# VITA-Group/SinNeRF

Measured on NVIDIA H100. Metric: rays/sec (64c+64f samples, 8x256 MLP), higher is better.
Workload: dtype fp32-parity: fp16 hi/lo split x3 on wgmma, fp32 accumulate

## Files before the change

### sinnerf_b200/csrc/field_tc.cu

```cuda
#include <stddef.h>
#include <stdlib.h>

#include <type_traits>
#include <utility>

#include "act16.cuh"
#include "common.cuh"
#include "wgmma.cuh"

namespace snb {
using namespace wg;

constexpr int kTile = 128;
constexpr int kNh = 128;
constexpr int kKc = 32;
constexpr uint32_t kStepBytes = kNh * 16 * 2;
constexpr int kWgs = 2;
constexpr int kThreads = (kWgs + 1) * 128;
constexpr int kProducerRegs = 24, kConsumerRegs = 240;
static_assert(128 * kProducerRegs + kWgs * 128 * kConsumerRegs <= 65536, "register file");
constexpr size_t kSmemOptIn = 232448;

enum { SRC_ENC = 0, SRC_HID = 1, SRC_DIR = 2 };

// ... 361 lines not shown
};

template <bool kBf16, bool kSplit, bool kEmbedded, int kTrain = 0>
__global__ void __launch_bounds__(kThreads, 1) field_tc_kernel(TcParams p) {
  static_assert(!(kTrain != 0 && kEmbedded), "the training forward is the fused (rays, z) entry only");
  using Smem = TcSmem<kSplit>;
  extern __shared__ unsigned char smem_raw[];
  Smem& s = *reinterpret_cast<Smem*>((reinterpret_cast<uintptr_t>(smem_raw) + 127) & ~uintptr_t(127));
  constexpr ConstLayout CL = make_const_layout();
  constexpr int kStages = Smem::kStages;
  constexpr int kParts = Smem::kParts;
  const ChunkTable& tab = c_chunks;
  const int tid = threadIdx.x, warp = tid >> 5, lane = tid & 31;
  const PackedHeader* hdr = reinterpret_cast<const PackedHeader*>(p.image);
  const int new_activation = hdr->new_activation;
  const float* g_cst = reinterpret_cast<const float*>(p.image + sizeof(PackedHeader));
  const unsigned char* g_chunks = p.image + sizeof(PackedHeader) + kConstBytes;
  const long long ntiles = (p.n_points + kTile - 1) / kTile;
  const int n_chunks = p.sigma_only ? tab.n_sigma_only : tab.n_total;

  if (tid == 0) {
    for (int i = 0; i < kStages; ++i) { mbar_init(&s.full[i], 1); mbar_init(&s.empty[i], kWgs * 4); }
    fence_mbar_init();
  }
  __syncthreads();

  if (warp >= kWgs * 4) {
    setmaxnreg_dec<kProducerRegs>();
    if (warp == kWgs * 4 && elect_one()) {
      const long long my_tiles = ntiles > (long long)blockIdx.x ? (ntiles - 1 - blockIdx.x) / gridDim.x + 1 : 0;
      const long long n_loads = my_tiles * n_chunks;
      uint32_t st = 0, ph = 0;
      int ci = 0;
      for (long long i = 0; i < n_loads; ++i) {
        mbar_wait(&s.empty[st], ph ^ 1);
        const Chunk c = tab.c[ci];
        const uint32_t bytes = kStepBytes * kParts * c.steps;
        mbar_arrive_expect_tx(&s.full[st], bytes);
        bulk_g2s(s.ring[st], g_chunks + (size_t)c.off * (kStepBytes * kParts), bytes, &s.full[st]);
        if (++ci == n_chunks) ci = 0;
        if (++st == kStages) { st = 0; ph ^= 1; }
      }
    }
    return;
  }
  setmaxnreg_inc<kConsumerRegs>();

  const int wgi = warp >> 2, wq = warp & 3, tq = lane & 3;
  const int r0 = wgi * 64 + wq * 16 + (lane >> 2);
  auto wg_sync = [&]() { named_bar_sync(1 + wgi, 128); };
  constexpr uint32_t kHidPart = kTile * kWidth * 2, kEncPart = kTile * kXyzPad * 2;
  constexpr uint32_t kOffRing = offsetof(Smem, ring), kOffHid = offsetof(Smem, hid), kOffEnc = offsetof(Smem, enc);
  const uint32_t sbase = smem_u32(&s);
  const uint32_t a_wg = sbase + wgi * 64 * 16;
  const uint32_t hid_thr = sbase + kOffHid + r0 * 16 + tq * 4;
  const int er = wgi * 64 + (tid & 63), epart = (tid >> 6) & 1;

  auto store_cell16 = [&](unsigned char* base, long long pt, int f8, int F, const float (&v)[8]) SNB_INLINE {
    if (pt >= p.ppad) return;
    const bool live = pt < p.n_points;
    uint4 c;
    c.x = live ? pack_half2_sat(v[0], v[1]) : 0u; c.y = live ? pack_half2_sat(v[2], v[3]) : 0u;
    c.z = live ? pack_half2_sat(v[4], v[5]) : 0u; c.w = live ? pack_half2_sat(v[6], v[7]) : 0u;
    *reinterpret_cast<uint4*>(base + a16_cell(pt, f8, F)) = c;
  };

  struct RowIn { float4 q0, q1; float z; };
  RowIn in{};
  auto load_row = [&](long long tile) SNB_INLINE {
    const long long pt = tile * kTile + er;
    if (!kEmbedded && tile < ntiles && pt < p.n_points) {
      const long long ray = pt / p.n_samples;
      in.q0 = *reinterpret_cast<const float4*>(p.rays + ray * 8);
      in.q1 = *reinterpret_cast<const float4*>(p.rays + ray * 8 + 4);
      in.z = p.z[pt];
    }
  };
  auto encode = [&](auto ltag, auto ptag, long long tile) SNB_INLINE {
    constexpr int L = decltype(ltag)::value, P = decltype(ptag)::value;
    constexpr bool kXyz = L == SNB_XYZ_FREQS;
    constexpr int kCh = 3 * (2 * L + 1), kPad = (kCh + 7) / 8 * 8, kK8 = kPad / 16;
    constexpr int c_lo = 8 * kK8 * P, c_hi = 8 * kK8 * (P + 1);
    const long long pt = tile * kTile + er;
    const bool live = pt < p.n_points;
    float v[kPad];
#pragma unroll
    for (int j = 0; j < kPad; ++j) v[j] = 0.f;
    if (kEmbedded) {
      const float* xr = p.x + pt * p.x_stride;
      const int nin = p.sigma_only ? kXyzCh : kXyzCh + kDirCh;
#pragma unroll
      for (int j = c_lo; j < (c_hi < kCh ? c_hi : kCh); ++j) {
        const int col = kXyz ? j : kXyzCh + j;
        v[j] = (live && col < nin) ? xr[col] : 0.f;
      }
    } else {
      float x[3] = {0.f, 0.f, 0.f};
      if (live) {
        if (kXyz) {
          x[0] = __fadd_rn(in.q0.x, __fmul_rn(in.q0.w, in.z));
          x[1] = __fadd_rn(in.q0.y, __fmul_rn(in.q1.x, in.z));
          x[2] = __fadd_rn(in.q0.z, __fmul_rn(in.q1.y, in.z));
        } else {
          x[0] = in.q0.w; x[1] = in.q1.x; x[2] = in.q1.y;
        }
      }
      v[0] = x[0]; v[1] = x[1]; v[2] = x[2];
#pragma unroll
      for (int f = 0; f < L; ++f)
#pragma unroll
        for (int c = 0; c < 3; ++c) {
          const int cs = 3 + 6 * f + c, cc = cs + 3;
          if ((cs >= c_lo && cs < c_hi) || (cc >= c_lo && cc < c_hi)) {
            float sn, cs_;
            if (kSplit) sincosf(x[c] * (float)(1 << f), &sn, &cs_);
            else sincos_fast(x[c] * (float)(1 << f), &sn, &cs_);
            v[cs] = sn;
            v[cc] = cs_;
          }
        }
    }
    static_for<kK8>([&](auto ktag) SNB_INLINE {
      constexpr int k8 = kK8 * P + decltype(ktag)::value;
      const float v8[8] = {v[8 * k8], v[8 * k8 + 1], v[8 * k8 + 2], v[8 * k8 + 3], v[8 * k8 + 4], v[8 * k8 + 5], v[8 * k8 + 6], v[8 * k8 + 7]};
      if (!kEmbedded) {
        if (kTrain == 1 && live) {
          float4* dst = reinterpret_cast<float4*>((kXyz ? p.save_enc + pt * kXyzPad : p.save_dir + pt * kDirPad) + k8 * 8);
          dst[0] = make_float4(v8[0], v8[1], v8[2], v8[3]); dst[1] = make_float4(v8[4], v8[5], v8[6], v8[7]);
        }
        if (kTrain == 2) store_cell16(kXyz ? p.a_enc : p.a_dir, pt, k8, kXyz ? kXyzPad : kDirPad, v8);
      }
      uint32_t h[4], l[4];
#pragma unroll
      for (int j = 0; j < 4; ++j) split_pair<kBf16, kSplit>(v8[2 * j], v8[2 * j + 1], h[j], l[j]);
      const uint32_t a = sbase + kOffEnc + k8 * (kTile * 16) + er * 16;
      st_shared_v4(a, h[0], h[1], h[2], h[3]);
      if (kSplit) st_shared_v4(a + kEncPart, l[0], l[1], l[2], l[3]);
    });
  };
  auto encode_rows = [&](auto ltag, long long tile) SNB_INLINE {
    if (epart == 0) encode(ltag, std::integral_constant<int, 0>{}, tile);
    else encode(ltag, std::integral_constant<int, 1>{}, tile);
  };

  auto mma = [&](float (&d)[64], uint64_t a, uint64_t b, bool first) SNB_INLINE {
    if (first) {
      if (kBf16) wgmma_m64n128_bf16_first(d, a, b);
      else wgmma_m64n128_f16_first(d, a, b);
    } else {
      if (kBf16) wgmma_m64n128_bf16(d, a, b, 1u);
      else wgmma_m64n128_f16(d, a, b, 1u);
    }
  };
  auto issue_step = [&](float (&d)[64], uint32_t ah, uint32_t al, uint32_t bh, uint32_t bl, bool first) SNB_INLINE {
    const uint64_t da_h = make_smem_desc(ah, kTile * 16, 128), db_h = make_smem_desc(bh, kNh * 16, 128);
    mma(d, da_h, db_h, first);
    if (kSplit) {
      mma(d, make_smem_desc(al, kTile * 16, 128), db_h, false);
      mma(d, da_h, make_smem_desc(bl, kNh * 16, 128), false);
    }
  };

  constexpr bool kDrained = kTrain != 0;
  float acc[2][64];
  float sig[2] = {0.f, 0.f};

  uint32_t st = 0, ph = 0;
  auto prev_stage = [&]() { return st == 0 ? (uint32_t)kStages - 1 : st - 1; };
  auto issue = [&](auto ctag) SNB_INLINE {
    constexpr int ci = decltype(ctag)::value;
    constexpr Chunk c = h_chunks.c[ci];
    float (&d)[64] = acc[c.half];
    mbar_wait(&s.full[st], ph);
    wgmma_fence();
    const uint32_t bh = sbase + kOffRing + st * Smem::kStageBytes, bl = bh + kStepBytes * c.steps;
    uint32_t abase;
    asm volatile("mov.b32 %0, %1;" : "=r"(abase) : "r"(a_wg));
    const uint32_t ah = abase + (c.src == SRC_HID ? kOffHid : kOffEnc) + c.a16 * 2 * (kTile * 16);
    constexpr uint32_t part = c.src == SRC_HID ? kHidPart : kEncPart;
    static_for<c.steps>([&](auto ktag) SNB_INLINE {
      constexpr int ks = decltype(ktag)::value;
      issue_step(d, ah + ks * 2 * (kTile * 16), ah + ks * 2 * (kTile * 16) + part, bh + ks * kStepBytes,
                 bl + ks * kStepBytes, ks == 0 && c.first);
    });
    wgmma_commit();
    if (kDrained ? !(c.first && c.half == 0) : ci != 0) {
      wgmma_wait<1>();
      if (lane == 0) mbar_arrive(&s.empty[prev_stage()]);
      __syncwarp();
    }
    if (++st == kStages) { st = 0; ph ^= 1; }
  };
  auto issue_range = [&](auto c0tag, auto ntag) SNB_INLINE {
    static_for<decltype(ntag)::value>([&](auto i) SNB_INLINE { issue(Int<decltype(c0tag)::value + decltype(i)::value>{}); });
  };
  auto drain = [&]() {
    wgmma_wait<0>();
    if (lane == 0) mbar_arrive(&s.empty[prev_stage()]);
    __syncwarp();
  };

  struct Block16 { uint32_t h16[4][2], mask[2]; };
  auto epi_block = [&](auto sigtag, auto htag, auto btag, int l, long long pt0) SNB_INLINE {
    constexpr bool kSigma = decltype(sigtag)::value;
    constexpr int h = decltype(htag)::value, b = decltype(btag)::value;
    const float* bias = g_cst + l * kWidth;
    const float (&d)[64] = acc[h];
    Block16 k16{};
    if (kSigma && h == 0 && b == 0) { sig[0] = 0.f; sig[1] = 0.f; }
    static_for<4>([&](auto jtag) SNB_INLINE {
      constexpr int jj = decltype(jtag)::value, j = 4 * b + jj;
      const int col = h * kNh + 8 * j + 2 * tq;
      const float2 bb = ldg_f2_here(bias + col);
#pragma unroll
      for (int rr = 0; rr < 2; ++rr) {
        float x0 = d[4 * j + 2 * rr] + bb.x, x1 = d[4 * j + 2 * rr + 1] + bb.y;
        uint32_t hi, lo;
        if (kTrain == 0 && !kSigma) {
          split_pair_relu<kBf16, kSplit>(x0, x1, hi, lo);
        } else {
          x0 = fmaxf(x0, 0.f); x1 = fmaxf(x1, 0.f);
          if (kSigma) {
            const float2 ww = ldg_f2_here(g_cst + CL.sigma_w + col);
            sig[rr] = fmaf(x0, ww.x, sig[rr]); sig[rr] = fmaf(x1, ww.y, sig[rr]);
          }
          split_pair<kBf16, kSplit, true>(x0, x1, hi, lo);
          const long long pt = pt0 + 8 * rr;
          if (kTrain == 1 && pt < p.n_points)
            *reinterpret_cast<float2*>(p.save_h + ((size_t)l * p.n_points + pt) * kWidth + col) = make_float2(x0, x1);
          if (kTrain == 2) {
            k16.h16[jj][rr] = kBf16 ? pack_half2_sat(x0, x1) : hi;
            k16.mask[rr] |= ((x0 > 0.f ? 1u : 0u) << (col & 31)) | ((x1 > 0.f ? 1u : 0u) << ((col & 31) + 1));
          }
        }
        const uint32_t a = hid_thr + (h * 16 + j) * (kTile * 16) + rr * 128;
        st_shared_u32(a, hi);
        if (kSplit) st_shared_u32(a + kHidPart, lo);
      }
    });
    if (kTrain == 2) {
#pragma unroll
      for (int rr = 0; rr < 2; ++rr) {
        k16.mask[rr] |= __shfl_xor_sync(0xffffffffu, k16.mask[rr], 1);
        k16.mask[rr] |= __shfl_xor_sync(0xffffffffu, k16.mask[rr], 2);
      }
    }
    return k16;
  };
  auto epi_half_end = [&]() SNB_INLINE {
    fence_proxy_async_smem();
    wg_sync();
  };
  auto sigma_head = [&](long long pt0) SNB_INLINE {
#pragma unroll
    for (int rr = 0; rr < 2; ++rr) {
      float v = sig[rr];
      v += __shfl_xor_sync(0xffffffffu, v, 1);
      v += __shfl_xor_sync(0xffffffffu, v, 2);
      sig[rr] = v + __ldg(g_cst + CL.sigma_b);
      const long long pt = pt0 + 8 * rr;
      if (p.sigma_only && tq == 0 && pt < p.n_points) p.out[pt] = sig[rr];
    }
  };

  auto dir_epilogue = [&](const float (&d)[64], long long pt0) SNB_INLINE {
    const float sh = new_activation ? 1.0f : 0.0f;
    float a[2][3] = {{0.f, 0.f, 0.f}, {0.f, 0.f, 0.f}};
#pragma unroll
    for (int j = 0; j < 16; ++j) {
      const int col = 8 * j + 2 * tq;
      const float2 bb = __ldg(reinterpret_cast<const float2*>(g_cst + CL.b[9] + col));
      const float2 w0 = __ldg(reinterpret_cast<const float2*>(g_cst + CL.rgb_w + col));
      const float2 w1 = __ldg(reinterpret_cast<const float2*>(g_cst + CL.rgb_w + kHalf + col));
      const float2 w2 = __ldg(reinterpret_cast<const float2*>(g_cst + CL.rgb_w + 2 * kHalf + col));
#pragma unroll
      for (int rr = 0; rr < 2; ++rr) {
        const long long pt = pt0 + 8 * rr;
        float x0 = d[4 * j + 2 * rr] + (bb.x - sh), x1 = d[4 * j + 2 * rr + 1] + (bb.y - sh);
        if (new_activation) { x0 = softplus_fast(x0); x1 = softplus_fast(x1); }
        else { x0 = fmaxf(x0, 0.f); x1 = fmaxf(x1, 0.f); }
        if (kTrain == 1 && pt < p.n_points) *reinterpret_cast<float2*>(p.save_g + pt * kHalf + col) = make_float2(x0, x1);
        if (kTrain == 2 && pt < p.ppad)
          *reinterpret_cast<uint32_t*>(p.a_g + a16_cell(pt, col >> 3, kHalf) + (col & 7) * 2) =
              pt < p.n_points ? pack_half2_sat(x0, x1) : 0u;
        a[rr][0] = fmaf(x1, w0.y, fmaf(x0, w0.x, a[rr][0]));
        a[rr][1] = fmaf(x1, w1.y, fmaf(x0, w1.x, a[rr][1]));
        a[rr][2] = fmaf(x1, w2.y, fmaf(x0, w2.x, a[rr][2]));
      }
    }
#pragma unroll
    for (int rr = 0; rr < 2; ++rr) {
      float c[3];
#pragma unroll
      for (int k = 0; k < 3; ++k) {
        float v = a[rr][k];
        v += __shfl_xor_sync(0xffffffffu, v, 1);
        v += __shfl_xor_sync(0xffffffffu, v, 2);
        v += __ldg(g_cst + CL.rgb_b + k);
        c[k] = new_activation ? widened_sigmoid_f(v) : sigmoid_f(v);
      }
      const long long pt = pt0 + 8 * rr;
      if (tq == 0 && pt < p.n_points) reinterpret_cast<float4*>(p.out)[pt] = make_float4(c[0], c[1], c[2], sig[rr]);
    }
  };

  auto trunk_epilogue = [&](auto ltag, int l, long long tile, long long pt0) SNB_INLINE {
    constexpr int L = decltype(ltag)::value;
    Block16 k16[2][4];
    static_for<2>([&](auto htag) SNB_INLINE {
      static_for<4>([&](auto btag) SNB_INLINE {
        k16[decltype(htag)::value][decltype(btag)::value] = epi_block(std::bool_constant<L == 7>{}, htag, btag, l, pt0);
      });
    });
    if (L == 7) sigma_head(pt0);
    if (L == 4 && !p.sigma_only) encode_rows(Int<SNB_DIR_FREQS>{}, tile);
    epi_half_end();
    if (kTrain == 2) {
      unsigned char* hb = p.a_h + (size_t)l * (size_t)p.ppad * (kWidth * 2);
#pragma unroll
      for (int rr = 0; rr < 2; ++rr) {
        const long long pt = pt0 + 8 * rr;
        if (pt >= p.ppad) continue;
        const bool live = pt < p.n_points;
#pragma unroll
        for (int h = 0; h < 2; ++h) {
#pragma unroll
          for (int j = 0; j < 16; ++j) {
            const int col = h * kNh + 8 * j + 2 * tq;
            *reinterpret_cast<uint32_t*>(hb + a16_cell(pt, col >> 3, kWidth) + (col & 7) * 2) =
                live ? k16[h][j / 4].h16[j % 4][rr] : 0u;
          }
#pragma unroll
          for (int b = 0; b < 4; ++b)
            if (tq == 0) p.a_mask[a16_mask_index(l, h * 4 + b, pt, p.ppad)] = live ? k16[h][b].mask[rr] : 0u;
        }
      }
// ... 161 lines not shown
```

### sinnerf_b200/csrc/wgmma.cuh

```cuda
#pragma once
#include <cuda_fp16.h>
#include <cuda_bf16.h>
#include <stdint.h>

namespace snb {
namespace wg {

__device__ __forceinline__ uint32_t smem_u32(const void* p) { return (uint32_t)__cvta_generic_to_shared(p); }

__device__ __forceinline__ bool elect_one() {
  uint32_t pred = 0;
  asm volatile(
      "{\n\t.reg .pred p;\n\t"
      "elect.sync _|p, 0xffffffff;\n\t"
      "selp.u32 %0, 1, 0, p;\n\t}"
      : "=r"(pred));
  return pred != 0;
}

__device__ __forceinline__ void mbar_init(uint64_t* bar, uint32_t count) {
  asm volatile("mbarrier.init.shared::cta.b64 [%0], %1;" ::"r"(smem_u32(bar)), "r"(count));
}
__device__ __forceinline__ void fence_mbar_init() { asm volatile("fence.mbarrier_init.release.cluster;" ::: "memory"); }
__device__ __forceinline__ void mbar_arrive(uint64_t* bar) {
  asm volatile("mbarrier.arrive.shared::cta.b64 _, [%0];" ::"r"(smem_u32(bar)) : "memory");
}
__device__ __forceinline__ void mbar_arrive_expect_tx(uint64_t* bar, uint32_t bytes) {
  asm volatile("mbarrier.arrive.expect_tx.shared::cta.b64 _, [%0], %1;" ::"r"(smem_u32(bar)), "r"(bytes) : "memory");
}
__device__ __forceinline__ bool mbar_try_wait(uint64_t* bar, uint32_t parity) {
  uint32_t ok;
  asm volatile(
      "{\n\t.reg .pred p;\n\t"
      "mbarrier.try_wait.parity.shared::cta.b64 p, [%1], %2;\n\t"
      "selp.u32 %0, 1, 0, p;\n\t}"
      : "=r"(ok)
      : "r"(smem_u32(bar)), "r"(parity)
      : "memory");
  return ok != 0;
}
__device__ __forceinline__ void mbar_wait(uint64_t* bar, uint32_t parity) {
  while (!mbar_try_wait(bar, parity)) {
  }
}

__device__ __forceinline__ void bulk_g2s(void* smem_dst, const void* gmem_src, uint32_t bytes, uint64_t* bar) {
  asm volatile("cp.async.bulk.shared::cluster.global.mbarrier::complete_tx::bytes [%0], [%1], %2, [%3];" ::"r"(
                   smem_u32(smem_dst)),
               "l"(gmem_src), "r"(bytes), "r"(smem_u32(bar))
               : "memory");
}

template <int N>
__device__ __forceinline__ void setmaxnreg_inc() { asm volatile("setmaxnreg.inc.sync.aligned.u32 %0;" ::"n"(N)); }
template <int N>
__device__ __forceinline__ void setmaxnreg_dec() { asm volatile("setmaxnreg.dec.sync.aligned.u32 %0;" ::"n"(N)); }

__device__ __forceinline__ void fence_proxy_async_smem() { asm volatile("fence.proxy.async.shared::cta;" ::: "memory"); }

__device__ __forceinline__ void st_shared_u32(uint32_t addr, uint32_t v) {
  asm volatile("st.shared.u32 [%0], %1;" ::"r"(addr), "r"(v));
}
__device__ __forceinline__ void st_shared_v4(uint32_t addr, uint32_t a, uint32_t b, uint32_t c, uint32_t d) {
  asm volatile("st.shared.v4.u32 [%0], {%1, %2, %3, %4};" ::"r"(addr), "r"(a), "r"(b), "r"(c), "r"(d));
}

__device__ __forceinline__ void named_bar_sync(int id, int count) {
  asm volatile("bar.sync %0, %1;" ::"r"(id), "r"(count) : "memory");
}

__device__ __forceinline__ uint64_t make_smem_desc(uint32_t smem_addr, uint32_t lbo_bytes, uint32_t sbo_bytes) {
  uint64_t d = 0;
  d |= (uint64_t)((smem_addr & 0x3FFFFu) >> 4);
  d |= (uint64_t)((lbo_bytes >> 4) & 0x3FFFu) << 16;
  d |= (uint64_t)((sbo_bytes >> 4) & 0x3FFFu) << 32;
  return d;
}

__device__ __forceinline__ void wgmma_fence() { asm volatile("wgmma.fence.sync.aligned;" ::: "memory"); }
__device__ __forceinline__ void wgmma_commit() { asm volatile("wgmma.commit_group.sync.aligned;" ::: "memory"); }
template <int N>
__device__ __forceinline__ void wgmma_wait() { asm volatile("wgmma.wait_group.sync.aligned %0;" ::"n"(N) : "memory"); }


__device__ __forceinline__ void wgmma_m64n128_f16(float (&d)[64], uint64_t a_desc, uint64_t b_desc, uint32_t accumulate) {
  asm volatile(
      "{\n\t.reg .pred p;\n\t"
      "setp.ne.b32 p, %66, 0;\n\t"
      "wgmma.mma_async.sync.aligned.m64n128k16.f32.f16.f16 "
      "{%0, %1, %2, %3, %4, %5, %6, %7, %8, %9, %10, %11, %12, %13, %14, %15, %16, %17, %18, %19, %20, %21, %22, %23, %24, %25, %26, %27, %28, %29, %30, %31, %32, %33, %34, %35, %36, %37, %38, %39, %40, %41, %42, %43, %44, %45, %46, %47, %48, %49, %50, %51, %52, %53, %54, %55, %56, %57, %58, %59, %60, %61, %62, %63}, %64, %65, p, 1, 1, 0, 0;\n\t}"
      : "+f"(d[0]), "+f"(d[1]), "+f"(d[2]), "+f"(d[3]), "+f"(d[4]), "+f"(d[5]), "+f"(d[6]), "+f"(d[7]), "+f"(d[8]), "+f"(d[9]), "+f"(d[10]), "+f"(d[11]), "+f"(d[12]), "+f"(d[13]), "+f"(d[14]), "+f"(d[15]), "+f"(d[16]), "+f"(d[17]), "+f"(d[18]), "+f"(d[19]), "+f"(d[20]), "+f"(d[21]), "+f"(d[22]), "+f"(d[23]), "+f"(d[24]), "+f"(d[25]), "+f"(d[26]), "+f"(d[27]), "+f"(d[28]), "+f"(d[29]), "+f"(d[30]), "+f"(d[31]), "+f"(d[32]), "+f"(d[33]), "+f"(d[34]), "+f"(d[35]), "+f"(d[36]), "+f"(d[37]), "+f"(d[38]), "+f"(d[39]), "+f"(d[40]), "+f"(d[41]), "+f"(d[42]), "+f"(d[43]), "+f"(d[44]), "+f"(d[45]), "+f"(d[46]), "+f"(d[47]), "+f"(d[48]), "+f"(d[49]), "+f"(d[50]), "+f"(d[51]), "+f"(d[52]), "+f"(d[53]), "+f"(d[54]), "+f"(d[55]), "+f"(d[56]), "+f"(d[57]), "+f"(d[58]), "+f"(d[59]), "+f"(d[60]), "+f"(d[61]), "+f"(d[62]), "+f"(d[63])
      : "l"(a_desc), "l"(b_desc), "r"(accumulate)
      : "memory");
}

__device__ __forceinline__ void wgmma_m64n128_bf16(float (&d)[64], uint64_t a_desc, uint64_t b_desc, uint32_t accumulate) {
  asm volatile(
      "{\n\t.reg .pred p;\n\t"
      "setp.ne.b32 p, %66, 0;\n\t"
      "wgmma.mma_async.sync.aligned.m64n128k16.f32.bf16.bf16 "
      "{%0, %1, %2, %3, %4, %5, %6, %7, %8, %9, %10, %11, %12, %13, %14, %15, %16, %17, %18, %19, %20, %21, %22, %23, %24, %25, %26, %27, %28, %29, %30, %31, %32, %33, %34, %35, %36, %37, %38, %39, %40, %41, %42, %43, %44, %45, %46, %47, %48, %49, %50, %51, %52, %53, %54, %55, %56, %57, %58, %59, %60, %61, %62, %63}, %64, %65, p, 1, 1, 0, 0;\n\t}"
      : "+f"(d[0]), "+f"(d[1]), "+f"(d[2]), "+f"(d[3]), "+f"(d[4]), "+f"(d[5]), "+f"(d[6]), "+f"(d[7]), "+f"(d[8]), "+f"(d[9]), "+f"(d[10]), "+f"(d[11]), "+f"(d[12]), "+f"(d[13]), "+f"(d[14]), "+f"(d[15]), "+f"(d[16]), "+f"(d[17]), "+f"(d[18]), "+f"(d[19]), "+f"(d[20]), "+f"(d[21]), "+f"(d[22]), "+f"(d[23]), "+f"(d[24]), "+f"(d[25]), "+f"(d[26]), "+f"(d[27]), "+f"(d[28]), "+f"(d[29]), "+f"(d[30]), "+f"(d[31]), "+f"(d[32]), "+f"(d[33]), "+f"(d[34]), "+f"(d[35]), "+f"(d[36]), "+f"(d[37]), "+f"(d[38]), "+f"(d[39]), "+f"(d[40]), "+f"(d[41]), "+f"(d[42]), "+f"(d[43]), "+f"(d[44]), "+f"(d[45]), "+f"(d[46]), "+f"(d[47]), "+f"(d[48]), "+f"(d[49]), "+f"(d[50]), "+f"(d[51]), "+f"(d[52]), "+f"(d[53]), "+f"(d[54]), "+f"(d[55]), "+f"(d[56]), "+f"(d[57]), "+f"(d[58]), "+f"(d[59]), "+f"(d[60]), "+f"(d[61]), "+f"(d[62]), "+f"(d[63])
      : "l"(a_desc), "l"(b_desc), "r"(accumulate)
      : "memory");
}

__device__ __forceinline__ void wgmma_m64n128_f16_first(float (&d)[64], uint64_t a_desc, uint64_t b_desc) {
  asm volatile(
      "{\n\t.reg .pred p;\n\t"
      "setp.ne.b32 p, %66, 0;\n\t"
      "wgmma.mma_async.sync.aligned.m64n128k16.f32.f16.f16 "
      "{%0, %1, %2, %3, %4, %5, %6, %7, %8, %9, %10, %11, %12, %13, %14, %15, %16, %17, %18, %19, %20, %21, %22, %23, %24, %25, %26, %27, %28, %29, %30, %31, %32, %33, %34, %35, %36, %37, %38, %39, %40, %41, %42, %43, %44, %45, %46, %47, %48, %49, %50, %51, %52, %53, %54, %55, %56, %57, %58, %59, %60, %61, %62, %63}, %64, %65, p, 1, 1, 0, 0;\n\t}"
      : "=f"(d[0]), "=f"(d[1]), "=f"(d[2]), "=f"(d[3]), "=f"(d[4]), "=f"(d[5]), "=f"(d[6]), "=f"(d[7]), "=f"(d[8]), "=f"(d[9]), "=f"(d[10]), "=f"(d[11]), "=f"(d[12]), "=f"(d[13]), "=f"(d[14]), "=f"(d[15]), "=f"(d[16]), "=f"(d[17]), "=f"(d[18]), "=f"(d[19]), "=f"(d[20]), "=f"(d[21]), "=f"(d[22]), "=f"(d[23]), "=f"(d[24]), "=f"(d[25]), "=f"(d[26]), "=f"(d[27]), "=f"(d[28]), "=f"(d[29]), "=f"(d[30]), "=f"(d[31]), "=f"(d[32]), "=f"(d[33]), "=f"(d[34]), "=f"(d[35]), "=f"(d[36]), "=f"(d[37]), "=f"(d[38]), "=f"(d[39]), "=f"(d[40]), "=f"(d[41]), "=f"(d[42]), "=f"(d[43]), "=f"(d[44]), "=f"(d[45]), "=f"(d[46]), "=f"(d[47]), "=f"(d[48]), "=f"(d[49]), "=f"(d[50]), "=f"(d[51]), "=f"(d[52]), "=f"(d[53]), "=f"(d[54]), "=f"(d[55]), "=f"(d[56]), "=f"(d[57]), "=f"(d[58]), "=f"(d[59]), "=f"(d[60]), "=f"(d[61]), "=f"(d[62]), "=f"(d[63])
      : "l"(a_desc), "l"(b_desc), "r"(0u)
      : "memory");
}

__device__ __forceinline__ void wgmma_m64n128_bf16_first(float (&d)[64], uint64_t a_desc, uint64_t b_desc) {
  asm volatile(
      "{\n\t.reg .pred p;\n\t"
      "setp.ne.b32 p, %66, 0;\n\t"
      "wgmma.mma_async.sync.aligned.m64n128k16.f32.bf16.bf16 "
      "{%0, %1, %2, %3, %4, %5, %6, %7, %8, %9, %10, %11, %12, %13, %14, %15, %16, %17, %18, %19, %20, %21, %22, %23, %24, %25, %26, %27, %28, %29, %30, %31, %32, %33, %34, %35, %36, %37, %38, %39, %40, %41, %42, %43, %44, %45, %46, %47, %48, %49, %50, %51, %52, %53, %54, %55, %56, %57, %58, %59, %60, %61, %62, %63}, %64, %65, p, 1, 1, 0, 0;\n\t}"
      : "=f"(d[0]), "=f"(d[1]), "=f"(d[2]), "=f"(d[3]), "=f"(d[4]), "=f"(d[5]), "=f"(d[6]), "=f"(d[7]), "=f"(d[8]), "=f"(d[9]), "=f"(d[10]), "=f"(d[11]), "=f"(d[12]), "=f"(d[13]), "=f"(d[14]), "=f"(d[15]), "=f"(d[16]), "=f"(d[17]), "=f"(d[18]), "=f"(d[19]), "=f"(d[20]), "=f"(d[21]), "=f"(d[22]), "=f"(d[23]), "=f"(d[24]), "=f"(d[25]), "=f"(d[26]), "=f"(d[27]), "=f"(d[28]), "=f"(d[29]), "=f"(d[30]), "=f"(d[31]), "=f"(d[32]), "=f"(d[33]), "=f"(d[34]), "=f"(d[35]), "=f"(d[36]), "=f"(d[37]), "=f"(d[38]), "=f"(d[39]), "=f"(d[40]), "=f"(d[41]), "=f"(d[42]), "=f"(d[43]), "=f"(d[44]), "=f"(d[45]), "=f"(d[46]), "=f"(d[47]), "=f"(d[48]), "=f"(d[49]), "=f"(d[50]), "=f"(d[51]), "=f"(d[52]), "=f"(d[53]), "=f"(d[54]), "=f"(d[55]), "=f"(d[56]), "=f"(d[57]), "=f"(d[58]), "=f"(d[59]), "=f"(d[60]), "=f"(d[61]), "=f"(d[62]), "=f"(d[63])
      : "l"(a_desc), "l"(b_desc), "r"(0u)
      : "memory");
}

__device__ __forceinline__ void wgmma_m64n256_f16_mn(float (&d)[128], uint64_t a_desc, uint64_t b_desc, uint32_t accumulate) {
  asm volatile(
      "{\n\t.reg .pred p;\n\t"
      "setp.ne.b32 p, %130, 0;\n\t"
      "wgmma.mma_async.sync.aligned.m64n256k16.f32.f16.f16 "
      "{%0, %1, %2, %3, %4, %5, %6, %7, %8, %9, %10, %11, %12, %13, %14, %15, %16, %17, %18, %19, %20, %21, %22, %23, %24, %25, %26, %27, %28, %29, %30, %31, %32, %33, %34, %35, %36, %37, %38, %39, %40, %41, %42, %43, %44, %45, %46, %47, %48, %49, %50, %51, %52, %53, %54, %55, %56, %57, %58, %59, %60, %61, %62, %63, %64, %65, %66, %67, %68, %69, %70, %71, %72, %73, %74, %75, %76, %77, %78, %79, %80, %81, %82, %83, %84, %85, %86, %87, %88, %89, %90, %91, %92, %93, %94, %95, %96, %97, %98, %99, %100, %101, %102, %103, %104, %105, %106, %107, %108, %109, %110, %111, %112, %113, %114, %115, %116, %117, %118, %119, %120, %121, %122, %123, %124, %125, %126, %127}, %128, %129, p, 1, 1, 1, 1;\n\t}"
      : "+f"(d[0]), "+f"(d[1]), "+f"(d[2]), "+f"(d[3]), "+f"(d[4]), "+f"(d[5]), "+f"(d[6]), "+f"(d[7]), "+f"(d[8]), "+f"(d[9]), "+f"(d[10]), "+f"(d[11]), "+f"(d[12]), "+f"(d[13]), "+f"(d[14]), "+f"(d[15]), "+f"(d[16]), "+f"(d[17]), "+f"(d[18]), "+f"(d[19]), "+f"(d[20]), "+f"(d[21]), "+f"(d[22]), "+f"(d[23]), "+f"(d[24]), "+f"(d[25]), "+f"(d[26]), "+f"(d[27]), "+f"(d[28]), "+f"(d[29]), "+f"(d[30]), "+f"(d[31]), "+f"(d[32]), "+f"(d[33]), "+f"(d[34]), "+f"(d[35]), "+f"(d[36]), "+f"(d[37]), "+f"(d[38]), "+f"(d[39]), "+f"(d[40]), "+f"(d[41]), "+f"(d[42]), "+f"(d[43]), "+f"(d[44]), "+f"(d[45]), "+f"(d[46]), "+f"(d[47]), "+f"(d[48]), "+f"(d[49]), "+f"(d[50]), "+f"(d[51]), "+f"(d[52]), "+f"(d[53]), "+f"(d[54]), "+f"(d[55]), "+f"(d[56]), "+f"(d[57]), "+f"(d[58]), "+f"(d[59]), "+f"(d[60]), "+f"(d[61]), "+f"(d[62]), "+f"(d[63]), "+f"(d[64]), "+f"(d[65]), "+f"(d[66]), "+f"(d[67]), "+f"(d[68]), "+f"(d[69]), "+f"(d[70]), "+f"(d[71]), "+f"(d[72]), "+f"(d[73]), "+f"(d[74]), "+f"(d[75]), "+f"(d[76]), "+f"(d[77]), "+f"(d[78]), "+f"(d[79]), "+f"(d[80]), "+f"(d[81]), "+f"(d[82]), "+f"(d[83]), "+f"(d[84]), "+f"(d[85]), "+f"(d[86]), "+f"(d[87]), "+f"(d[88]), "+f"(d[89]), "+f"(d[90]), "+f"(d[91]), "+f"(d[92]), "+f"(d[93]), "+f"(d[94]), "+f"(d[95]), "+f"(d[96]), "+f"(d[97]), "+f"(d[98]), "+f"(d[99]), "+f"(d[100]), "+f"(d[101]), "+f"(d[102]), "+f"(d[103]), "+f"(d[104]), "+f"(d[105]), "+f"(d[106]), "+f"(d[107]), "+f"(d[108]), "+f"(d[109]), "+f"(d[110]), "+f"(d[111]), "+f"(d[112]), "+f"(d[113]), "+f"(d[114]), "+f"(d[115]), "+f"(d[116]), "+f"(d[117]), "+f"(d[118]), "+f"(d[119]), "+f"(d[120]), "+f"(d[121]), "+f"(d[122]), "+f"(d[123]), "+f"(d[124]), "+f"(d[125]), "+f"(d[126]), "+f"(d[127])
      : "l"(a_desc), "l"(b_desc), "r"(accumulate)
      : "memory");
}

__device__ __forceinline__ void wgmma_m64n128_f16_mn(float (&d)[64], uint64_t a_desc, uint64_t b_desc, uint32_t accumulate) {
  asm volatile(
      "{\n\t.reg .pred p;\n\t"
      "setp.ne.b32 p, %66, 0;\n\t"
      "wgmma.mma_async.sync.aligned.m64n128k16.f32.f16.f16 "
      "{%0, %1, %2, %3, %4, %5, %6, %7, %8, %9, %10, %11, %12, %13, %14, %15, %16, %17, %18, %19, %20, %21, %22, %23, %24, %25, %26, %27, %28, %29, %30, %31, %32, %33, %34, %35, %36, %37, %38, %39, %40, %41, %42, %43, %44, %45, %46, %47, %48, %49, %50, %51, %52, %53, %54, %55, %56, %57, %58, %59, %60, %61, %62, %63}, %64, %65, p, 1, 1, 1, 1;\n\t}"
      : "+f"(d[0]), "+f"(d[1]), "+f"(d[2]), "+f"(d[3]), "+f"(d[4]), "+f"(d[5]), "+f"(d[6]), "+f"(d[7]), "+f"(d[8]), "+f"(d[9]), "+f"(d[10]), "+f"(d[11]), "+f"(d[12]), "+f"(d[13]), "+f"(d[14]), "+f"(d[15]), "+f"(d[16]), "+f"(d[17]), "+f"(d[18]), "+f"(d[19]), "+f"(d[20]), "+f"(d[21]), "+f"(d[22]), "+f"(d[23]), "+f"(d[24]), "+f"(d[25]), "+f"(d[26]), "+f"(d[27]), "+f"(d[28]), "+f"(d[29]), "+f"(d[30]), "+f"(d[31]), "+f"(d[32]), "+f"(d[33]), "+f"(d[34]), "+f"(d[35]), "+f"(d[36]), "+f"(d[37]), "+f"(d[38]), "+f"(d[39]), "+f"(d[40]), "+f"(d[41]), "+f"(d[42]), "+f"(d[43]), "+f"(d[44]), "+f"(d[45]), "+f"(d[46]), "+f"(d[47]), "+f"(d[48]), "+f"(d[49]), "+f"(d[50]), "+f"(d[51]), "+f"(d[52]), "+f"(d[53]), "+f"(d[54]), "+f"(d[55]), "+f"(d[56]), "+f"(d[57]), "+f"(d[58]), "+f"(d[59]), "+f"(d[60]), "+f"(d[61]), "+f"(d[62]), "+f"(d[63])
      : "l"(a_desc), "l"(b_desc), "r"(accumulate)
      : "memory");
}

__device__ __forceinline__ void wgmma_m64n64_f16_mn(float (&d)[32], uint64_t a_desc, uint64_t b_desc, uint32_t accumulate) {
  asm volatile(
      "{\n\t.reg .pred p;\n\t"
      "setp.ne.b32 p, %34, 0;\n\t"
      "wgmma.mma_async.sync.aligned.m64n64k16.f32.f16.f16 "
      "{%0, %1, %2, %3, %4, %5, %6, %7, %8, %9, %10, %11, %12, %13, %14, %15, %16, %17, %18, %19, %20, %21, %22, %23, %24, %25, %26, %27, %28, %29, %30, %31}, %32, %33, p, 1, 1, 1, 1;\n\t}"
      : "+f"(d[0]), "+f"(d[1]), "+f"(d[2]), "+f"(d[3]), "+f"(d[4]), "+f"(d[5]), "+f"(d[6]), "+f"(d[7]), "+f"(d[8]), "+f"(d[9]), "+f"(d[10]), "+f"(d[11]), "+f"(d[12]), "+f"(d[13]), "+f"(d[14]), "+f"(d[15]), "+f"(d[16]), "+f"(d[17]), "+f"(d[18]), "+f"(d[19]), "+f"(d[20]), "+f"(d[21]), "+f"(d[22]), "+f"(d[23]), "+f"(d[24]), "+f"(d[25]), "+f"(d[26]), "+f"(d[27]), "+f"(d[28]), "+f"(d[29]), "+f"(d[30]), "+f"(d[31])
      : "l"(a_desc), "l"(b_desc), "r"(accumulate)
      : "memory");
}

__device__ __forceinline__ void wgmma_m64n32_f16_mn(float (&d)[16], uint64_t a_desc, uint64_t b_desc, uint32_t accumulate) {
  asm volatile(
      "{\n\t.reg .pred p;\n\t"
      "setp.ne.b32 p, %18, 0;\n\t"
      "wgmma.mma_async.sync.aligned.m64n32k16.f32.f16.f16 "
      "{%0, %1, %2, %3, %4, %5, %6, %7, %8, %9, %10, %11, %12, %13, %14, %15}, %16, %17, p, 1, 1, 1, 1;\n\t}"
      : "+f"(d[0]), "+f"(d[1]), "+f"(d[2]), "+f"(d[3]), "+f"(d[4]), "+f"(d[5]), "+f"(d[6]), "+f"(d[7]), "+f"(d[8]), "+f"(d[9]), "+f"(d[10]), "+f"(d[11]), "+f"(d[12]), "+f"(d[13]), "+f"(d[14]), "+f"(d[15])
      : "l"(a_desc), "l"(b_desc), "r"(accumulate)
      : "memory");
}

__device__ __forceinline__ void wgmma_m64n128_f16_rs(float (&d)[64], const uint32_t (&a)[4], uint64_t b_desc, uint32_t accumulate) {
  asm volatile(
      "{\n\t.reg .pred p;\n\t"
      "setp.ne.b32 p, %69, 0;\n\t"
      "wgmma.mma_async.sync.aligned.m64n128k16.f32.f16.f16 "
      "{%0, %1, %2, %3, %4, %5, %6, %7, %8, %9, %10, %11, %12, %13, %14, %15, %16, %17, %18, %19, %20, %21, %22, %23, %24, %25, %26, %27, %28, %29, %30, %31, %32, %33, %34, %35, %36, %37, %38, %39, %40, %41, %42, %43, %44, %45, %46, %47, %48, %49, %50, %51, %52, %53, %54, %55, %56, %57, %58, %59, %60, %61, %62, %63}, {%64, %65, %66, %67}, %68, p, 1, 1, 0;\n\t}"
      : "+f"(d[0]), "+f"(d[1]), "+f"(d[2]), "+f"(d[3]), "+f"(d[4]), "+f"(d[5]), "+f"(d[6]), "+f"(d[7]), "+f"(d[8]), "+f"(d[9]), "+f"(d[10]), "+f"(d[11]), "+f"(d[12]), "+f"(d[13]), "+f"(d[14]), "+f"(d[15]), "+f"(d[16]), "+f"(d[17]), "+f"(d[18]), "+f"(d[19]), "+f"(d[20]), "+f"(d[21]), "+f"(d[22]), "+f"(d[23]), "+f"(d[24]), "+f"(d[25]), "+f"(d[26]), "+f"(d[27]), "+f"(d[28]), "+f"(d[29]), "+f"(d[30]), "+f"(d[31]), "+f"(d[32]), "+f"(d[33]), "+f"(d[34]), "+f"(d[35]), "+f"(d[36]), "+f"(d[37]), "+f"(d[38]), "+f"(d[39]), "+f"(d[40]), "+f"(d[41]), "+f"(d[42]), "+f"(d[43]), "+f"(d[44]), "+f"(d[45]), "+f"(d[46]), "+f"(d[47]), "+f"(d[48]), "+f"(d[49]), "+f"(d[50]), "+f"(d[51]), "+f"(d[52]), "+f"(d[53]), "+f"(d[54]), "+f"(d[55]), "+f"(d[56]), "+f"(d[57]), "+f"(d[58]), "+f"(d[59]), "+f"(d[60]), "+f"(d[61]), "+f"(d[62]), "+f"(d[63])
      : "r"(a[0]), "r"(a[1]), "r"(a[2]), "r"(a[3]), "l"(b_desc), "r"(accumulate)
      : "memory");
}

__device__ __forceinline__ void wgmma_m64n256_bf16_mn(float (&d)[128], uint64_t a_desc, uint64_t b_desc, uint32_t accumulate) {
  asm volatile(
      "{\n\t.reg .pred p;\n\t"
      "setp.ne.b32 p, %130, 0;\n\t"
      "wgmma.mma_async.sync.aligned.m64n256k16.f32.bf16.bf16 "
      "{%0, %1, %2, %3, %4, %5, %6, %7, %8, %9, %10, %11, %12, %13, %14, %15, %16, %17, %18, %19, %20, %21, %22, %23, %24, %25, %26, %27, %28, %29, %30, %31, %32, %33, %34, %35, %36, %37, %38, %39, %40, %41, %42, %43, %44, %45, %46, %47, %48, %49, %50, %51, %52, %53, %54, %55, %56, %57, %58, %59, %60, %61, %62, %63, %64, %65, %66, %67, %68, %69, %70, %71, %72, %73, %74, %75, %76, %77, %78, %79, %80, %81, %82, %83, %84, %85, %86, %87, %88, %89, %90, %91, %92, %93, %94, %95, %96, %97, %98, %99, %100, %101, %102, %103, %104, %105, %106, %107, %108, %109, %110, %111, %112, %113, %114, %115, %116, %117, %118, %119, %120, %121, %122, %123, %124, %125, %126, %127}, %128, %129, p, 1, 1, 1, 1;\n\t}"
      : "+f"(d[0]), "+f"(d[1]), "+f"(d[2]), "+f"(d[3]), "+f"(d[4]), "+f"(d[5]), "+f"(d[6]), "+f"(d[7]), "+f"(d[8]), "+f"(d[9]), "+f"(d[10]), "+f"(d[11]), "+f"(d[12]), "+f"(d[13]), "+f"(d[14]), "+f"(d[15]), "+f"(d[16]), "+f"(d[17]), "+f"(d[18]), "+f"(d[19]), "+f"(d[20]), "+f"(d[21]), "+f"(d[22]), "+f"(d[23]), "+f"(d[24]), "+f"(d[25]), "+f"(d[26]), "+f"(d[27]), "+f"(d[28]), "+f"(d[29]), "+f"(d[30]), "+f"(d[31]), "+f"(d[32]), "+f"(d[33]), "+f"(d[34]), "+f"(d[35]), "+f"(d[36]), "+f"(d[37]), "+f"(d[38]), "+f"(d[39]), "+f"(d[40]), "+f"(d[41]), "+f"(d[42]), "+f"(d[43]), "+f"(d[44]), "+f"(d[45]), "+f"(d[46]), "+f"(d[47]), "+f"(d[48]), "+f"(d[49]), "+f"(d[50]), "+f"(d[51]), "+f"(d[52]), "+f"(d[53]), "+f"(d[54]), "+f"(d[55]), "+f"(d[56]), "+f"(d[57]), "+f"(d[58]), "+f"(d[59]), "+f"(d[60]), "+f"(d[61]), "+f"(d[62]), "+f"(d[63]), "+f"(d[64]), "+f"(d[65]), "+f"(d[66]), "+f"(d[67]), "+f"(d[68]), "+f"(d[69]), "+f"(d[70]), "+f"(d[71]), "+f"(d[72]), "+f"(d[73]), "+f"(d[74]), "+f"(d[75]), "+f"(d[76]), "+f"(d[77]), "+f"(d[78]), "+f"(d[79]), "+f"(d[80]), "+f"(d[81]), "+f"(d[82]), "+f"(d[83]), "+f"(d[84]), "+f"(d[85]), "+f"(d[86]), "+f"(d[87]), "+f"(d[88]), "+f"(d[89]), "+f"(d[90]), "+f"(d[91]), "+f"(d[92]), "+f"(d[93]), "+f"(d[94]), "+f"(d[95]), "+f"(d[96]), "+f"(d[97]), "+f"(d[98]), "+f"(d[99]), "+f"(d[100]), "+f"(d[101]), "+f"(d[102]), "+f"(d[103]), "+f"(d[104]), "+f"(d[105]), "+f"(d[106]), "+f"(d[107]), "+f"(d[108]), "+f"(d[109]), "+f"(d[110]), "+f"(d[111]), "+f"(d[112]), "+f"(d[113]), "+f"(d[114]), "+f"(d[115]), "+f"(d[116]), "+f"(d[117]), "+f"(d[118]), "+f"(d[119]), "+f"(d[120]), "+f"(d[121]), "+f"(d[122]), "+f"(d[123]), "+f"(d[124]), "+f"(d[125]), "+f"(d[126]), "+f"(d[127])
      : "l"(a_desc), "l"(b_desc), "r"(accumulate)
      : "memory");
}

__device__ __forceinline__ void wgmma_m64n64_bf16_mn(float (&d)[32], uint64_t a_desc, uint64_t b_desc, uint32_t accumulate) {
  asm volatile(
      "{\n\t.reg .pred p;\n\t"
      "setp.ne.b32 p, %34, 0;\n\t"
      "wgmma.mma_async.sync.aligned.m64n64k16.f32.bf16.bf16 "
      "{%0, %1, %2, %3, %4, %5, %6, %7, %8, %9, %10, %11, %12, %13, %14, %15, %16, %17, %18, %19, %20, %21, %22, %23, %24, %25, %26, %27, %28, %29, %30, %31}, %32, %33, p, 1, 1, 1, 1;\n\t}"
      : "+f"(d[0]), "+f"(d[1]), "+f"(d[2]), "+f"(d[3]), "+f"(d[4]), "+f"(d[5]), "+f"(d[6]), "+f"(d[7]), "+f"(d[8]), "+f"(d[9]), "+f"(d[10]), "+f"(d[11]), "+f"(d[12]), "+f"(d[13]), "+f"(d[14]), "+f"(d[15]), "+f"(d[16]), "+f"(d[17]), "+f"(d[18]), "+f"(d[19]), "+f"(d[20]), "+f"(d[21]), "+f"(d[22]), "+f"(d[23]), "+f"(d[24]), "+f"(d[25]), "+f"(d[26]), "+f"(d[27]), "+f"(d[28]), "+f"(d[29]), "+f"(d[30]), "+f"(d[31])
      : "l"(a_desc), "l"(b_desc), "r"(accumulate)
      : "memory");
}

__device__ __forceinline__ void wgmma_m64n32_bf16_mn(float (&d)[16], uint64_t a_desc, uint64_t b_desc, uint32_t accumulate) {
  asm volatile(
      "{\n\t.reg .pred p;\n\t"
      "setp.ne.b32 p, %18, 0;\n\t"
      "wgmma.mma_async.sync.aligned.m64n32k16.f32.bf16.bf16 "
      "{%0, %1, %2, %3, %4, %5, %6, %7, %8, %9, %10, %11, %12, %13, %14, %15}, %16, %17, p, 1, 1, 1, 1;\n\t}"
      : "+f"(d[0]), "+f"(d[1]), "+f"(d[2]), "+f"(d[3]), "+f"(d[4]), "+f"(d[5]), "+f"(d[6]), "+f"(d[7]), "+f"(d[8]), "+f"(d[9]), "+f"(d[10]), "+f"(d[11]), "+f"(d[12]), "+f"(d[13]), "+f"(d[14]), "+f"(d[15])
      : "l"(a_desc), "l"(b_desc), "r"(accumulate)
      : "memory");
}

__device__ __forceinline__ void wgmma_m64n64_f16(float (&d)[32], uint64_t a_desc, uint64_t b_desc) {
  asm volatile(
      "wgmma.mma_async.sync.aligned.m64n64k16.f32.f16.f16 "
      "{%0, %1, %2, %3, %4, %5, %6, %7, %8, %9, %10, %11, %12, %13, %14, %15, %16, %17, %18, %19, %20, %21, %22, %23, %24, %25, %26, %27, %28, %29, %30, %31}, %32, %33, 1, 1, 1, 0, 0;"
      : "+f"(d[0]), "+f"(d[1]), "+f"(d[2]), "+f"(d[3]), "+f"(d[4]), "+f"(d[5]), "+f"(d[6]), "+f"(d[7]), "+f"(d[8]), "+f"(d[9]), "+f"(d[10]), "+f"(d[11]), "+f"(d[12]), "+f"(d[13]), "+f"(d[14]), "+f"(d[15]), "+f"(d[16]), "+f"(d[17]), "+f"(d[18]), "+f"(d[19]), "+f"(d[20]), "+f"(d[21]), "+f"(d[22]), "+f"(d[23]), "+f"(d[24]), "+f"(d[25]), "+f"(d[26]), "+f"(d[27]), "+f"(d[28]), "+f"(d[29]), "+f"(d[30]), "+f"(d[31])
      : "l"(a_desc), "l"(b_desc)
      : "memory");
}

__device__ __forceinline__ void wgmma_m64n64_bf16(float (&d)[32], uint64_t a_desc, uint64_t b_desc) {
  asm volatile(
      "wgmma.mma_async.sync.aligned.m64n64k16.f32.bf16.bf16 "
      "{%0, %1, %2, %3, %4, %5, %6, %7, %8, %9, %10, %11, %12, %13, %14, %15, %16, %17, %18, %19, %20, %21, %22, %23, %24, %25, %26, %27, %28, %29, %30, %31}, %32, %33, 1, 1, 1, 0, 0;"
      : "+f"(d[0]), "+f"(d[1]), "+f"(d[2]), "+f"(d[3]), "+f"(d[4]), "+f"(d[5]), "+f"(d[6]), "+f"(d[7]), "+f"(d[8]), "+f"(d[9]), "+f"(d[10]), "+f"(d[11]), "+f"(d[12]), "+f"(d[13]), "+f"(d[14]), "+f"(d[15]), "+f"(d[16]), "+f"(d[17]), "+f"(d[18]), "+f"(d[19]), "+f"(d[20]), "+f"(d[21]), "+f"(d[22]), "+f"(d[23]), "+f"(d[24]), "+f"(d[25]), "+f"(d[26]), "+f"(d[27]), "+f"(d[28]), "+f"(d[29]), "+f"(d[30]), "+f"(d[31])
      : "l"(a_desc), "l"(b_desc)
      : "memory");
}

__device__ __forceinline__ void wgmma_m64n128_bf16_rs(float (&d)[64], const uint32_t (&a)[4], uint64_t b_desc, uint32_t accumulate) {
  asm volatile(
      "{\n\t.reg .pred p;\n\t"
      "setp.ne.b32 p, %69, 0;\n\t"
      "wgmma.mma_async.sync.aligned.m64n128k16.f32.bf16.bf16 "
      "{%0, %1, %2, %3, %4, %5, %6, %7, %8, %9, %10, %11, %12, %13, %14, %15, %16, %17, %18, %19, %20, %21, %22, %23, %24, %25, %26, %27, %28, %29, %30, %31, %32, %33, %34, %35, %36, %37, %38, %39, %40, %41, %42, %43, %44, %45, %46, %47, %48, %49, %50, %51, %52, %53, %54, %55, %56, %57, %58, %59, %60, %61, %62, %63}, {%64, %65, %66, %67}, %68, p, 1, 1, 0;\n\t}"
      : "+f"(d[0]), "+f"(d[1]), "+f"(d[2]), "+f"(d[3]), "+f"(d[4]), "+f"(d[5]), "+f"(d[6]), "+f"(d[7]), "+f"(d[8]), "+f"(d[9]), "+f"(d[10]), "+f"(d[11]), "+f"(d[12]), "+f"(d[13]), "+f"(d[14]), "+f"(d[15]), "+f"(d[16]), "+f"(d[17]), "+f"(d[18]), "+f"(d[19]), "+f"(d[20]), "+f"(d[21]), "+f"(d[22]), "+f"(d[23]), "+f"(d[24]), "+f"(d[25]), "+f"(d[26]), "+f"(d[27]), "+f"(d[28]), "+f"(d[29]), "+f"(d[30]), "+f"(d[31]), "+f"(d[32]), "+f"(d[33]), "+f"(d[34]), "+f"(d[35]), "+f"(d[36]), "+f"(d[37]), "+f"(d[38]), "+f"(d[39]), "+f"(d[40]), "+f"(d[41]), "+f"(d[42]), "+f"(d[43]), "+f"(d[44]), "+f"(d[45]), "+f"(d[46]), "+f"(d[47]), "+f"(d[48]), "+f"(d[49]), "+f"(d[50]), "+f"(d[51]), "+f"(d[52]), "+f"(d[53]), "+f"(d[54]), "+f"(d[55]), "+f"(d[56]), "+f"(d[57]), "+f"(d[58]), "+f"(d[59]), "+f"(d[60]), "+f"(d[61]), "+f"(d[62]), "+f"(d[63])
      : "r"(a[0]), "r"(a[1]), "r"(a[2]), "r"(a[3]), "l"(b_desc), "r"(accumulate)
      : "memory");
}

}
}
```

Baseline: 1.131 million.

## Load split A fragments into registers via ldmatrix and use register-sourced wgmma

For the fp16 hi/lo split path, the activation (A) tiles are now loaded once per chunk into registers with ldmatrix before waiting on the weight stage. The three wgmma products then take A from registers (RS form) instead of reading A twice from shared memory through descriptors. Issuing the loads early lets them overlap the mbarrier wait and cuts shared-memory traffic for A. In exchange, each consumer thread holds 8 extra registers per k-step in a kernel already capped at 240 registers, so spills are possible. The ldmatrix fragment layout must also match what RS wgmma expects, or results will be wrong.

```diff
diff --git a/sinnerf_b200/csrc/field_tc.cu b/sinnerf_b200/csrc/field_tc.cu
--- a/sinnerf_b200/csrc/field_tc.cu
+++ b/sinnerf_b200/csrc/field_tc.cu
@@ -537,14 +537,16 @@
       else wgmma_m64n128_f16(d, a, b, 1u);
     }
   };
-  auto issue_step = [&](float (&d)[64], uint32_t ah, uint32_t al, uint32_t bh, uint32_t bl, bool first) SNB_INLINE {
-    const uint64_t da_h = make_smem_desc(ah, kTile * 16, 128), db_h = make_smem_desc(bh, kNh * 16, 128);
-    mma(d, da_h, db_h, first);
-    if (kSplit) {
-      mma(d, make_smem_desc(al, kTile * 16, 128), db_h, false);
-      mma(d, da_h, make_smem_desc(bl, kNh * 16, 128), false);
-    }
-  };
+  auto mma_rs = [&](float (&d)[64], const uint32_t (&a)[4], uint64_t b, bool first) SNB_INLINE {
+    if (first) {
+      if (kBf16) wgmma_m64n128_bf16_rs_first(d, a, b);
+      else wgmma_m64n128_f16_rs_first(d, a, b);
+    } else {
+      if (kBf16) wgmma_m64n128_bf16_rs(d, a, b, 1u);
+      else wgmma_m64n128_f16_rs(d, a, b, 1u);
+    }
+  };
+  const uint32_t a_frag = a_wg + (wq * 16 + (lane & 15)) * 16 + (lane >> 4) * (kTile * 16);
 
   constexpr bool kDrained = kTrain != 0;
   float acc[2][64];
@@ -556,17 +558,33 @@
     constexpr int ci = decltype(ctag)::value;
     constexpr Chunk c = h_chunks.c[ci];
     float (&d)[64] = acc[c.half];
+    uint32_t abase;
+    asm volatile("mov.b32 %0, %1;" : "=r"(abase) : "r"(kSplit ? a_frag : a_wg));
+    const uint32_t ah = abase + (c.src == SRC_HID ? kOffHid : kOffEnc) + c.a16 * 2 * (kTile * 16);
+    [[maybe_unused]] uint32_t fh[kSplit ? c.steps : 1][4], fl[kSplit ? c.steps : 1][4];
+    if constexpr (kSplit) {
+      constexpr uint32_t part = c.src == SRC_HID ? kHidPart : kEncPart;
+      static_for<c.steps>([&](auto ktag) SNB_INLINE {
+        constexpr int ks = decltype(ktag)::value;
+        ldmatrix_x4(fh[ks], ah + ks * 2 * (kTile * 16));
+        ldmatrix_x4(fl[ks], ah + ks * 2 * (kTile * 16) + part);
+      });
+    }
     mbar_wait(&s.full[st], ph);
     wgmma_fence();
-    const uint32_t bh = sbase + kOffRing + st * Smem::kStageBytes, bl = bh + kStepBytes * c.steps;
-    uint32_t abase;
-    asm volatile("mov.b32 %0, %1;" : "=r"(abase) : "r"(a_wg));
-    const uint32_t ah = abase + (c.src == SRC_HID ? kOffHid : kOffEnc) + c.a16 * 2 * (kTile * 16);
-    constexpr uint32_t part = c.src == SRC_HID ? kHidPart : kEncPart;
+    const uint32_t bh = sbase + kOffRing + st * Smem::kStageBytes;
     static_for<c.steps>([&](auto ktag) SNB_INLINE {
       constexpr int ks = decltype(ktag)::value;
-      issue_step(d, ah + ks * 2 * (kTile * 16), ah + ks * 2 * (kTile * 16) + part, bh + ks * kStepBytes,
-                 bl + ks * kStepBytes, ks == 0 && c.first);
+      constexpr bool first = ks == 0 && c.first;
+      const uint64_t db_h = make_smem_desc(bh + ks * kStepBytes, kNh * 16, 128);
+      if constexpr (kSplit) {
+        const uint32_t bl = bh + kStepBytes * (c.steps + ks);
+        mma_rs(d, fh[ks], db_h, first);
+        mma_rs(d, fl[ks], db_h, false);
+        mma_rs(d, fh[ks], make_smem_desc(bl, kNh * 16, 128), false);
+      } else {
+        mma(d, make_smem_desc(ah + ks * 2 * (kTile * 16), kTile * 16, 128), db_h, first);
+      }
     });
     wgmma_commit();
     if (kDrained ? !(c.first && c.half == 0) : ci != 0) {
diff --git a/sinnerf_b200/csrc/wgmma.cuh b/sinnerf_b200/csrc/wgmma.cuh
--- a/sinnerf_b200/csrc/wgmma.cuh
+++ b/sinnerf_b200/csrc/wgmma.cuh
@@ -63,6 +63,12 @@
 }
 __device__ __forceinline__ void st_shared_v4(uint32_t addr, uint32_t a, uint32_t b, uint32_t c, uint32_t d) {
   asm volatile("st.shared.v4.u32 [%0], {%1, %2, %3, %4};" ::"r"(addr), "r"(a), "r"(b), "r"(c), "r"(d));
+}
+
+__device__ __forceinline__ void ldmatrix_x4(uint32_t (&r)[4], uint32_t addr) {
+  asm volatile("ldmatrix.sync.aligned.m8n8.x4.shared.b16 {%0, %1, %2, %3}, [%4];"
+               : "=r"(r[0]), "=r"(r[1]), "=r"(r[2]), "=r"(r[3])
+               : "r"(addr));
 }
 
 __device__ __forceinline__ void named_bar_sync(int id, int count) {
@@ -244,5 +250,27 @@
       : "memory");
 }
 
-}
-}
+__device__ __forceinline__ void wgmma_m64n128_f16_rs_first(float (&d)[64], const uint32_t (&a)[4], uint64_t b_desc) {
+  asm volatile(
+      "{\n\t.reg .pred p;\n\t"
+      "setp.ne.b32 p, %69, 0;\n\t"
+      "wgmma.mma_async.sync.aligned.m64n128k16.f32.f16.f16 "
+      "{%0, %1, %2, %3, %4, %5, %6, %7, %8, %9, %10, %11, %12, %13, %14, %15, %16, %17, %18, %19, %20, %21, %22, %23, %24, %25, %26, %27, %28, %29, %30, %31, %32, %33, %34, %35, %36, %37, %38, %39, %40, %41, %42, %43, %44, %45, %46, %47, %48, %49, %50, %51, %52, %53, %54, %55, %56, %57, %58, %59, %60, %61, %62, %63}, {%64, %65, %66, %67}, %68, p, 1, 1, 0;\n\t}"
+      : "=f"(d[0]), "=f"(d[1]), "=f"(d[2]), "=f"(d[3]), "=f"(d[4]), "=f"(d[5]), "=f"(d[6]), "=f"(d[7]), "=f"(d[8]), "=f"(d[9]), "=f"(d[10]), "=f"(d[11]), "=f"(d[12]), "=f"(d[13]), "=f"(d[14]), "=f"(d[15]), "=f"(d[16]), "=f"(d[17]), "=f"(d[18]), "=f"(d[19]), "=f"(d[20]), "=f"(d[21]), "=f"(d[22]), "=f"(d[23]), "=f"(d[24]), "=f"(d[25]), "=f"(d[26]), "=f"(d[27]), "=f"(d[28]), "=f"(d[29]), "=f"(d[30]), "=f"(d[31]), "=f"(d[32]), "=f"(d[33]), "=f"(d[34]), "=f"(d[35]), "=f"(d[36]), "=f"(d[37]), "=f"(d[38]), "=f"(d[39]), "=f"(d[40]), "=f"(d[41]), "=f"(d[42]), "=f"(d[43]), "=f"(d[44]), "=f"(d[45]), "=f"(d[46]), "=f"(d[47]), "=f"(d[48]), "=f"(d[49]), "=f"(d[50]), "=f"(d[51]), "=f"(d[52]), "=f"(d[53]), "=f"(d[54]), "=f"(d[55]), "=f"(d[56]), "=f"(d[57]), "=f"(d[58]), "=f"(d[59]), "=f"(d[60]), "=f"(d[61]), "=f"(d[62]), "=f"(d[63])
+      : "r"(a[0]), "r"(a[1]), "r"(a[2]), "r"(a[3]), "l"(b_desc), "r"(0u)
+      : "memory");
+}
+
+__device__ __forceinline__ void wgmma_m64n128_bf16_rs_first(float (&d)[64], const uint32_t (&a)[4], uint64_t b_desc) {
+  asm volatile(
+      "{\n\t.reg .pred p;\n\t"
+      "setp.ne.b32 p, %69, 0;\n\t"
+      "wgmma.mma_async.sync.aligned.m64n128k16.f32.bf16.bf16 "
+      "{%0, %1, %2, %3, %4, %5, %6, %7, %8, %9, %10, %11, %12, %13, %14, %15, %16, %17, %18, %19, %20, %21, %22, %23, %24, %25, %26, %27, %28, %29, %30, %31, %32, %33, %34, %35, %36, %37, %38, %39, %40, %41, %42, %43, %44, %45, %46, %47, %48, %49, %50, %51, %52, %53, %54, %55, %56, %57, %58, %59, %60, %61, %62, %63}, {%64, %65, %66, %67}, %68, p, 1, 1, 0;\n\t}"
+      : "=f"(d[0]), "=f"(d[1]), "=f"(d[2]), "=f"(d[3]), "=f"(d[4]), "=f"(d[5]), "=f"(d[6]), "=f"(d[7]), "=f"(d[8]), "=f"(d[9]), "=f"(d[10]), "=f"(d[11]), "=f"(d[12]), "=f"(d[13]), "=f"(d[14]), "=f"(d[15]), "=f"(d[16]), "=f"(d[17]), "=f"(d[18]), "=f"(d[19]), "=f"(d[20]), "=f"(d[21]), "=f"(d[22]), "=f"(d[23]), "=f"(d[24]), "=f"(d[25]), "=f"(d[26]), "=f"(d[27]), "=f"(d[28]), "=f"(d[29]), "=f"(d[30]), "=f"(d[31]), "=f"(d[32]), "=f"(d[33]), "=f"(d[34]), "=f"(d[35]), "=f"(d[36]), "=f"(d[37]), "=f"(d[38]), "=f"(d[39]), "=f"(d[40]), "=f"(d[41]), "=f"(d[42]), "=f"(d[43]), "=f"(d[44]), "=f"(d[45]), "=f"(d[46]), "=f"(d[47]), "=f"(d[48]), "=f"(d[49]), "=f"(d[50]), "=f"(d[51]), "=f"(d[52]), "=f"(d[53]), "=f"(d[54]), "=f"(d[55]), "=f"(d[56]), "=f"(d[57]), "=f"(d[58]), "=f"(d[59]), "=f"(d[60]), "=f"(d[61]), "=f"(d[62]), "=f"(d[63])
+      : "r"(a[0]), "r"(a[1]), "r"(a[2]), "r"(a[3]), "l"(b_desc), "r"(0u)
+      : "memory");
+}
+
+}
+}
```

New measurement: 1.129 million (median of 6 runs). About the same (-0.2%).
